# matthewdm0816/BridgeQA

Hardware: AMD Instinct MI355X
Metric: train samples/s (40k-pt scene + 512^2 view, bs16) (higher is better)
Workload: dtype bf16

## Files before the change

bridgeqa_amd/_ext.py:

```python
import ctypes
import os

import torch

_LIB_PATH = os.environ.get("BQHIP_LIB") or os.path.join(os.path.dirname(os.path.abspath(__file__)), "lib", "libbqhip.so")

if not os.path.exists(_LIB_PATH):
    raise ImportError(
        "bridgeqa_amd: %s is missing -- build it with `python -m bridgeqa_amd.build` "
        "(hipcc --offload-arch=gfx950). There is no CPU fallback." % _LIB_PATH)

_lib = ctypes.CDLL(_LIB_PATH)
_lib.bq_last_error.restype = ctypes.c_char_p
_lib.bq_abi_version.restype = ctypes.c_int
ABI_VERSION = 6
if _lib.bq_abi_version() != ABI_VERSION:
    raise ImportError("bridgeqa_amd: libbqhip.so ABI %d != %d (stale library: python -m bridgeqa_amd.build --force)"
                      % (_lib.bq_abi_version(), ABI_VERSION))

_vp, _i, _f = ctypes.c_void_p, ctypes.c_int, ctypes.c_float
_SIGS = {
    "bq_opt_n_threads": [_i],
    "bq_furthest_point_sampling": [_vp, _vp, ctypes.c_size_t, _vp, _i, _i, _i, _vp],
    "bq_furthest_point_sampling_bruteforce": [_vp, _vp, _vp, _i, _i, _i, _vp],
# ... 906 lines not shown
        n_cs = Nj if (pxc and qxc and f32) else Ni
        if epilogue != EPI_BIAS_CE and colsum is not None and (colsum.dtype != torch.float32 or colsum.numel() != n_cs
                                                               or not colsum.is_contiguous()):
            raise RuntimeError("gemm: colsum must be a contiguous fp32 (%d,) tensor" % n_cs)
        for t, nm in ((out2, "out2"), (aux, "aux")):
            if epilogue != EPI_BIAS_CE and t is not None and (t.dtype != torch.bfloat16 or t.shape != out.shape
                                                              or t.stride() != out.stride()):
                raise RuntimeError("gemm: %s must be bf16 and laid out like out" % nm)
        d.bias, d.out2, d.aux, d.colsum = _p(bias), _p(out2), _p(aux), _p(colsum)
        d.ldp, d.ldq, d.ldo = P.stride(0), ldq, ldo
        d.q_rpb, d.q_bstride, d.o_rpb, d.o_bstride = q_rpb, q_bs, o_rpb, o_bs
        d.accum = int(bool(pr.get("accum", False)))
        d.Ni, d.Nj, d.Kc = Ni, Nj, Kc
        d.p_bytes, d.q_bytes, d.ksplit = int(pr.get("p_bytes", 0)), int(pr.get("q_bytes", 0)), int(pr.get("ksplit", 1))
        if "Kc" in pr:
            d.Kc = int(pr["Kc"])
        mid_ok = (not qxc and not f32 and d.Kc >= 128 and colsum is None
                  and epilogue in (EPI_NONE, EPI_BIAS, EPI_BIAS_GELU, EPI_DGELU, EPI_ADD))
        all_mid_ok = mid_ok if k == 0 else (all_mid_ok and mid_ok)
        t_auto = max(t_auto, pick_tile(Ni, Nj, qxc, True))
    if t_auto == 128 and not all_mid_ok:
        t_auto = 256
    if (t_auto == 128 and TILE256_MIN_K[0] and not pxc and epilogue in (EPI_NONE, EPI_BIAS)
            and all(int(arr[k].Kc) >= TILE256_MIN_K[0] for k in range(n))):
        t_auto = 256
    if t_auto == 256 and any_map and tile is None and not (pxc and qxc and f32):
        t_auto = 64
    dev = problems[0]["out"].device
    if (tile or t_auto) != 128:
        flags &= ~GEMM_BACKGROUND
    with torch.cuda.device(dev):
        if (tile or t_auto) == 128 and n == 1 and (STREAMK[0] or STREAMK256[0]):
            _streamk_workspace(dev)
        _check(_lib.bq_gemm_bf16(arr, n, int(flags), int(epilogue), int(tile or t_auto), _stream()), "gemm_bf16")


def _gemm_grouped_det(problems, flags, epilogue, tile):
    if STREAMK[0] or STREAMK256[0]:
        raise RuntimeError("gemm: stream-K is on (streamk_enable / streamk256_enable) while the deterministic mode is on")
    f32 = bool(flags & GEMM_OUT_F32)
    probs, folds, sums = [], [], []
    for pr in problems:
        ks = int(pr.get("ksplit", 1))
        if epilogue != EPI_BIAS_CE and ks > 1:
            out = pr["out"]
            if not f32 or pr.get("colsum") is not None or pr.get("accum") or out.dim() != 2 or out.stride(1) != 1:
                raise RuntimeError("gemm: a cut contraction in the deterministic mode needs fp32 plain-row out, no colsum or accum")
            slab = torch.empty(ks, out.shape[0], out.stride(0), dtype=torch.float32, device=out.device)
            folds.append((slab, out, ks))
            pr = dict(pr, out=slab[0, :, :out.shape[1]])
        elif not f32 and epilogue != EPI_BIAS_CE and pr.get("colsum") is not None:
            sums.append((pr["out"], pr["colsum"]))
            pr = dict(pr, colsum=None)
        probs.append(pr)
    _gemm_grouped_launch(probs, flags | GEMM_DET, epilogue, tile)
    for slab, out, ks in folds:
        R, C = out.shape
        with torch.cuda.device(out.device):
            _check(_det_entry("gemm_splitk_fold")(_p(slab), _p(out), None, ks, R, C, out.stride(0), _stream()),
                   "gemm_splitk_fold_det")
    if sums:
        _colsum_grouped_into([o.reshape(-1, o.shape[-1]) if o.dim() == 3 else o for o, _ in sums], [c for _, c in sums],
                             "gemm_epilogue_colsum")


STREAMK = [False]
STREAMK256 = [os.environ.get("BQ_GEMM_STREAMK256", "0") == "1"]
_SK_WS = {}
_lib.bq_gemm_workspace_bytes.restype = ctypes.c_long
_lib.bq_gemm_set_workspace.argtypes = [_vp, ctypes.c_long, _vp]
_lib.bq_gemm_set_workspace.restype = ctypes.c_int
_lib.bq_gemm_streamk_mode.argtypes = [_i]
_lib.bq_gemm_streamk_mode.restype = ctypes.c_int


def _streamk_apply():
    on = STREAMK[0] or STREAMK256[0]
    _lib.bq_gemm_streamk_mode((1 if STREAMK[0] else 0) | (2 if STREAMK256[0] else 0))
    for (d, sp), (ws, st) in _SK_WS.items():
        with torch.cuda.device(d):
            _check(_lib.bq_gemm_set_workspace(_p(ws) if on else None, ws.numel() if on else 0, sp), "gemm_set_workspace")


def streamk_enable(flag):
    STREAMK[0] = bool(flag)
    _streamk_apply()


def streamk256_enable(flag):
    STREAMK256[0] = bool(flag)
    _streamk_apply()


_streamk_apply()


def _streamk_workspace(dev):
    st = torch.cuda.current_stream(dev)
    key = (dev.index if dev.index is not None else torch.cuda.current_device(), st.cuda_stream)
    if key in _SK_WS or torch.cuda.is_current_stream_capturing():
        return
    nbytes = int(_lib.bq_gemm_workspace_bytes())
    ws = torch.zeros(nbytes, dtype=torch.uint8, device=dev)
    _check(_lib.bq_gemm_set_workspace(_p(ws), nbytes, st.cuda_stream), "gemm_set_workspace")
    _SK_WS[key] = (ws, st)


def gemm_fwd(x, w, bias=None, gelu=False, tile=None, out=None, background=False):
    _mat(x, "x"), _mat(w, "w")
    M, N = x.shape[0], w.shape[0]
    with torch.cuda.device(x.device):
        y = torch.empty(M, N, dtype=torch.bfloat16, device=x.device) if out is None else out
        act = torch.empty_like(y) if gelu else None
    epi = EPI_BIAS_GELU if gelu else (EPI_BIAS if bias is not None else EPI_NONE)
    gemm_grouped([dict(P=w, Q=x, out=y, bias=bias, out2=act)], GEMM_BACKGROUND if background else 0, epi, tile)
    return (y, act) if gelu else y


def gemm_dx(dy, w, pre_act=None, colsum=None, tile=None, add=None, background=False, wt=None):
    _mat(dy, "dy"), _mat(w, "w")
    M, K = dy.shape[0], w.shape[1]
    if pre_act is not None and add is not None:
        raise RuntimeError("gemm_dx: pre_act and add are exclusive")
    if wt is not None and (colsum is not None or tuple(wt.shape) != (K, w.shape[0])):
        wt = None
    with torch.cuda.device(dy.device):
        dx = torch.empty(M, K, dtype=torch.bfloat16, device=dy.device)
    gemm_grouped([dict(P=w if wt is None else wt, Q=dy, out=dx, aux=pre_act if add is None else add, colsum=colsum)],
                 (GEMM_P_XC if wt is None else 0) | (GEMM_BACKGROUND if background else 0),
                 EPI_DGELU if pre_act is not None else (EPI_ADD if add is not None else EPI_NONE), tile)
    return dx


def gemm_dw(dy, x, tile=None):
    _mat(dy, "dy"), _mat(x, "x")
    N, K = dy.shape[1], x.shape[1]
    with torch.cuda.device(dy.device):
        dw = torch.empty(N, K, dtype=torch.float32, device=dy.device)
    gemm_grouped([dict(P=x, Q=dy, out=dw)], GEMM_P_XC | GEMM_Q_XC | GEMM_OUT_F32, EPI_NONE, tile)
    return dw


class _ColsumDesc(ctypes.Structure):
    _fields_ = [("g", _vp), ("out", _vp), ("M", _i), ("N", _i), ("ld", _i)]


_lib.bq_colsum_grouped_bf16.argtypes = [ctypes.POINTER(_ColsumDesc), _i, _vp]
_lib.bq_colsum_grouped_bf16.restype = ctypes.c_int


_lib.bq_colsum_grouped_det_floats.argtypes = [ctypes.POINTER(_ColsumDesc), _i]
_lib.bq_colsum_grouped_det_floats.restype = _l
_lib.bq_colsum_grouped_det_bf16.argtypes = [ctypes.POINTER(_ColsumDesc), _i, _vp, _vp]
_lib.bq_colsum_grouped_det_bf16.restype = ctypes.c_int


def _colsum_grouped_into(mats, outs, site):
    n = len(mats)
    arr = (_ColsumDesc * n)()
    for k, (m, o) in enumerate(zip(mats, outs)):
        _mat(m, "g")
        if m.dtype != torch.bfloat16 or o.dtype != torch.float32 or not o.is_contiguous() or o.numel() != m.shape[1]:
            raise RuntimeError("colsum_grouped: bf16 (M, N) matrices into contiguous fp32 (N,) sums")
        arr[k].g, arr[k].out, arr[k].M, arr[k].N, arr[k].ld = m.data_ptr(), o.data_ptr(), m.shape[0], m.shape[1], m.stride(0)
    dev = mats[0].device
    with torch.cuda.device(dev):
# ... 483 lines not shown
```

bridgeqa_amd/csrc/gemm_common.h:

```cpp
#pragma once
#include <type_traits>

#include "bq_common.h"
#include "bqhip_fusion.h"

namespace bq {

typedef __bf16 bf16x8 __attribute__((ext_vector_type(8)));
typedef __bf16 bf16x4 __attribute__((ext_vector_type(4)));
typedef float f32x4 __attribute__((ext_vector_type(4)));
typedef __attribute__((address_space(3))) bf16x4 lds_bf16x4_t;
typedef __attribute__((address_space(3))) void lds_void_t;

enum { EPI_NONE = 0, EPI_BIAS = 1, EPI_BIAS_GELU = 2, EPI_DGELU = 3, EPI_BIAS_CE = 4, EPI_ADD = 5 };
enum { GF_P_XC = 1, GF_Q_XC = 2, GF_OUT_F32 = 4, GF_ACCUM = 8 };

struct GemmProblem {
  const __bf16 *P, *Q;
  void *out;
  const void *bias;
  void *out2;
  const __bf16 *aux;
  float *colsum;
  int ldp, ldq, ldo;
  int Ni, Nj, Kc;
  int tile0;
  unsigned p_bytes, q_bytes;
  int q_bstride, o_bstride;
  int rpb_pack;
  int tiles_ks;
  int flags;
  __host__ __device__ __forceinline__ int q_rpb() const { return rpb_pack & 0xffff; }
  __host__ __device__ __forceinline__ int o_rpb() const { return (int)((unsigned)rpb_pack >> 16); }
  __host__ __device__ __forceinline__ int tiles_i() const { return tiles_ks & 0xffff; }
  __host__ __device__ __forceinline__ int ksplit() const { return (int)((unsigned)tiles_ks >> 16); }
  __host__ __device__ __forceinline__ int bias_bf16() const { return flags & 1; }
  __host__ __device__ __forceinline__ int accum() const { return (flags >> 1) & 1; }
};
static_assert(sizeof(GemmProblem) == 112, "GemmProblem grew: GEMM_MAX_PROBLEMS x sizeof must stay below the 4 KB kernarg limit");

__device__ __forceinline__ unsigned mapped_row(int r, int ld, int rpb, int bstride) {
  if (rpb == 0) return (unsigned)(r * ld);
  const int b = r / rpb;
  return (unsigned)(b * bstride + (r - b * rpb) * ld);
}

__device__ __forceinline__ void load_bias4(const GemmProblem &pr, int i, float (&bv)[4]) {
  if (pr.bias_bf16()) {
    const bf16x4 b = *reinterpret_cast<const bf16x4 *>(reinterpret_cast<const __bf16 *>(pr.bias) + i);
    bv[0] = (float)b[0]; bv[1] = (float)b[1]; bv[2] = (float)b[2]; bv[3] = (float)b[3];
  } else {
    const float4 b = *reinterpret_cast<const float4 *>(reinterpret_cast<const float *>(pr.bias) + i);
    bv[0] = b.x; bv[1] = b.y; bv[2] = b.z; bv[3] = b.w;
  }
}

constexpr int GEMM_MAX_PROBLEMS = 36;
struct GemmArgs {
  int n;
  int total_tiles;
  GemmProblem p[GEMM_MAX_PROBLEMS];
  void *sk_ws;
};
constexpr long SK_TICKET_BYTES = 65536, SK_SLAB_BYTES = 256 * 128 * 4;
static_assert(sizeof(GemmArgs) <= 4096, "kernel-argument limit");

__device__ __forceinline__ int xg(int kc) { return ((kc >> 1) & 1) | (((kc >> 3) & 1) << 1); }

constexpr float GELU_A1 = 1.59525515f, GELU_A3 = 7.38511083e-2f, GELU_A5 = -6.82350683e-4f;
__device__ __forceinline__ float gauss_cdf(float x, float &x2) {
  const float xc = __builtin_amdgcn_fmed3f(x, -8.0f, 8.0f);
  x2 = xc * xc;
  constexpr float L = -1.4426950408889634f;
  const float z = xc * __builtin_fmaf(x2, __builtin_fmaf(x2, GELU_A5 * L, GELU_A3 * L), GELU_A1 * L);
  return __builtin_amdgcn_rcpf(1.0f + __builtin_amdgcn_exp2f(z));
}
__device__ __forceinline__ float gelu_f(float x) {
  float x2;
  return x * gauss_cdf(x, x2);
}
__device__ __forceinline__ float dgelu_f(float x) {
  const float xc = __builtin_amdgcn_fmed3f(x, -8.0f, 8.0f);
  const float x2 = xc * xc;
  constexpr float L = -1.4426950408889634f;
  const float z = xc * __builtin_fmaf(x2, __builtin_fmaf(x2, GELU_A5 * L, GELU_A3 * L), GELU_A1 * L);
  const float s = __builtin_amdgcn_rcpf(1.0f + __builtin_amdgcn_exp2f(z));
  const float u = xc * __builtin_fmaf(x2, __builtin_fmaf(x2, 5.0f * GELU_A5, 3.0f * GELU_A3), GELU_A1);
  const float v = __builtin_fmaf(-s, s, s);
  return __builtin_fmaf(u, v, s);
}

constexpr unsigned GELU_TAB_LO = (127 - 16) << 7, GELU_TAB_HI = (127 + 3) << 7;
constexpr int GELU_TAB_HALF = (int)(GELU_TAB_HI - GELU_TAB_LO) + 1, GELU_TAB_N = 2 * GELU_TAB_HALF;
template <bool DERIV>
__device__ __forceinline__ void gelu_tab_fill(float *tab, int tid, int nthreads) {
  for (int e = tid; e < GELU_TAB_N; e += nthreads) {
    const unsigned sgn = e >= GELU_TAB_HALF ? 1u : 0u;
    const unsigned bits = (sgn << 15) | ((unsigned)e - sgn * GELU_TAB_HALF + GELU_TAB_LO);
    const float x = __uint_as_float(bits << 16);
    float x2;
    tab[e] = DERIV ? dgelu_f(x) : gauss_cdf(x, x2);
  }
}
__device__ __forceinline__ float gelu_tab_at(const float *tab, unsigned bits16) {
  const unsigned mag = min(max(bits16 & 0x7fffu, GELU_TAB_LO), GELU_TAB_HI) - GELU_TAB_LO;
  return tab[mag + ((bits16 >> 15) & 1u) * GELU_TAB_HALF];
}

template <int CTRL>
__device__ __forceinline__ float dpp_f32_add(float v) {
  return __int_as_float(__builtin_amdgcn_update_dpp(0, __float_as_int(v), CTRL, 0xF, 0xF, true));
}

__device__ __forceinline__ unsigned pack_bf16x2(float a, float b) {
  typedef __bf16 bf16x2_t __attribute__((ext_vector_type(2)));
  bf16x2_t v = {(__bf16)a, (__bf16)b};
  return __builtin_bit_cast(unsigned, v);
}

template <bool XC>
__device__ __forceinline__ bf16x8 read_frag(const unsigned char *unit, int sub16, int kk, int kc_base, const int (&xc_base)[4]) {
  if (!XC) {
    return *reinterpret_cast<const bf16x8 *>(unit + sub16 * 2048 + (kc_base ^ (kk << 6)));
  } else {
    const unsigned char *a0 = unit + xc_base[sub16] + kk * 4096;
    const bf16x4 lo = __builtin_amdgcn_ds_read_tr16_b64_v4bf16((lds_bf16x4_t *)a0);
    const bf16x4 hi = __builtin_amdgcn_ds_read_tr16_b64_v4bf16((lds_bf16x4_t *)(a0 + 512));
    return __builtin_shufflevector(lo, hi, 0, 1, 2, 3, 4, 5, 6, 7);
  }
}

template <bool XC>
__device__ __forceinline__ bf16x8 read_frag_cf(const unsigned char *unit, int sub16, int kk, int kc_base, int xc0, int xcg) {
  if (!XC) {
    return *reinterpret_cast<const bf16x8 *>(unit + sub16 * 2048 + (kc_base ^ (kk << 6)));
  } else {
    const unsigned char *a0 = unit + xc0 + ((sub16 ^ xcg) << 5) + kk * 4096;
    const bf16x4 lo = __builtin_amdgcn_ds_read_tr16_b64_v4bf16((lds_bf16x4_t *)a0);
    const bf16x4 hi = __builtin_amdgcn_ds_read_tr16_b64_v4bf16((lds_bf16x4_t *)(a0 + 512));
    return __builtin_shufflevector(lo, hi, 0, 1, 2, 3, 4, 5, 6, 7);
  }
}

template <bool XC>
__device__ __forceinline__ bf16x8 read_frag(const unsigned char *unit, int sub16, int kk, int kc_base, const int (&xc_base)[4]);
// ... 77 lines not shown
```

bridgeqa_amd/csrc/gemm_mid.hip:

```cpp
#include "gemm_common.h"

#ifndef BQ_MID_ABLATE
#define BQ_MID_ABLATE 0
#endif

namespace bq {

typedef __attribute__((address_space(3))) unsigned char lds_u8_t;
typedef unsigned u32x2_t __attribute__((ext_vector_type(2)));
typedef unsigned u32x4_t __attribute__((ext_vector_type(4)));

template <bool P_XC, bool Q_XC, int EPI, bool OUT_F32, int ST_AUX, bool SK = false>
__global__ __launch_bounds__(256, 2) void gemm128_kernel(const GemmArgs args) {
  static_assert(!OUT_F32 || (P_XC && Q_XC && EPI == EPI_NONE), "fp32 out = the weight-gradient form");
  static_assert(!Q_XC || OUT_F32, "a contraction-major Q = the weight-gradient form");
  static_assert(!SK || (!OUT_F32 && EPI != EPI_BIAS_GELU), "stream-K: bf16 out, one output");
  __shared__ __attribute__((aligned(16))) unsigned char smem[65536 + 4 * 2048 + (SK ? 16 : 0)];
  const int tid = threadIdx.x;
  const int lane = tid & 63;
  const int wave = __builtin_amdgcn_readfirstlane(tid >> 6);
  const int wr = wave >> 1, wc = wave & 1;
  const int nwg = args.total_tiles, G = (int)gridDim.x;

  const int row16 = lane & 15, q4 = lane >> 4, cp = lane & 7, lr = lane >> 3;
  const int kc_base = row16 * 128 + ((q4 ^ (row16 & 7)) << 4);
  const int xc_q = (lane & 15) >> 2;
  const int xcg = (xc_q >> 1) | ((q4 & 1) << 1), xc0 = (8 * q4 + xc_q) * 128 + 8 * (lane & 3);
  constexpr int PA0 = 0, PA1 = 16384, QB = 32768;
  const int uA0 = PA0 + wr * 8192, uA1 = PA1 + wr * 8192;
  const int bsub = wc * 2;

  struct Tile { int pi, i0, j0, nkt, kt0, t; };
  auto xcd_order = [](int v, int n) {
    const int q = n >> 3, r = n & 7, x = v & 7;
    return (x < r ? x * (q + 1) : r * (q + 1) + (x - r) * q) + (v >> 3);
  };
  auto decode_t = [&](int t) {
    int pi = 0;
    for (int k = 1; k < args.n; ++k)
      if (t >= args.p[k].tile0) pi = k;
    const GemmProblem &pr = args.p[pi];
    const int tl = t - pr.tile0;
    const int tiles_j = (pr.Nj + 127) >> 7;
    Tile tt;
    tt.pi = pi;
    tt.j0 = (tiles_j - 1 - tl / pr.tiles_i()) * 128;
    tt.i0 = (tl % pr.tiles_i()) * 256;
    tt.nkt = (pr.Kc + 63) >> 6;
    tt.kt0 = 0;
    tt.t = t;
    return tt;
  };
  auto decode = [&](int v) { return decode_t(xcd_order(v, nwg)); };
  const int nkt_full = SK ? (args.p[0].Kc + 63) >> 6 : 1;
  const int U = SK ? nwg * nkt_full : 0;
  auto bound = [&](int x) {
    int b = (int)((long)x * U / G);
    const int r = b % nkt_full;
    return r == 1 ? b - 1 : (r == nkt_full - 1 ? b + 1 : b);
  };
  auto seg = [&](int u, int ue) {
    const int t = u / nkt_full;
    Tile tt = decode_t(t);
    tt.kt0 = u - t * nkt_full;
    const int left = nkt_full - tt.kt0;
    tt.nkt = left < ue - u ? left : ue - u;
    return tt;
  };
  const int slot = SK ? xcd_order((int)blockIdx.x, G) : 0;
  int su = SK ? bound(slot) : 0;
  const int sue = SK ? bound(slot + 1) : 0;

  unsigned vP[2], vQ[2];
  unsigned stepP[2], dgP[2], ddP[2], ddQ[2], stepQ[2];
  int remP[2], remQ[2];
  int rsrcP_pi[2], rsrcQ_pi[2];
  const unsigned DEAD = 0x80000000u;
  const int ur0 = wave * 8 + lr;

  auto set_p = [&](int half, const Tile &tt, bool live) {
    const GemmProblem &pr = args.p[tt.pi];
    const int ldp = pr.ldp;
    unsigned v;
    if (!P_XC) v = (unsigned)(((tt.i0 + half * 64 + ur0) * ldp + (cp ^ (ur0 & 7)) * 8) * 2);
    else v = (unsigned)((ur0 * ldp + tt.i0 + half * 64 + (cp ^ (xg(ur0) << 1)) * 8) * 2);
    stepP[half] = P_XC ? (unsigned)(64 * ldp * 2) : 128u;
    if (SK) v += (unsigned)tt.kt0 * stepP[half];
    vP[half] = live ? v : DEAD;
    dgP[half] = P_XC ? 256u : (unsigned)(128 * ldp * 2);
    ddP[half] = (unsigned)(32 * ldp * 2);
    remP[half] = live ? tt.nkt : 0x40000000;
    rsrcP_pi[half] = tt.pi;
  };
  auto set_q = [&](int half, const Tile &tt, bool live) {
    const GemmProblem &pr = args.p[tt.pi];
    unsigned v;
    if (!Q_XC) {
      const int row0 = tt.j0 + half * 32 + ur0;
      const unsigned o0 = mapped_row(row0, pr.ldq, pr.q_rpb(), pr.q_bstride);
      v = (o0 + (unsigned)((cp ^ (ur0 & 7)) * 8)) * 2u;
      ddQ[half] = pr.q_rpb() ? (mapped_row(row0 + 64, pr.ldq, pr.q_rpb(), pr.q_bstride) - o0) * 2u : (unsigned)(64 * pr.ldq * 2);
    } else {
      const int c = cp ^ (xg(ur0) << 1);
      v = (unsigned)((ur0 * pr.ldq + tt.j0 + (c >> 2) * 64 + half * 32 + (c & 3) * 8) * 2);
      ddQ[half] = (unsigned)(32 * pr.ldq * 2);
    }
    stepQ[half] = Q_XC ? (unsigned)(64 * pr.ldq * 2) : 128u;
    if (SK) v += (unsigned)tt.kt0 * stepQ[half];
    vQ[half] = live ? v : DEAD;
    remQ[half] = live ? tt.nkt : 0x40000000;
    rsrcQ_pi[half] = tt.pi;
  };

  int v = blockIdx.x;
  Tile cur = SK ? seg(su, sue) : decode(v);
  bool has_next = SK ? (su + cur.nkt < sue) : (v + G < nwg);
  Tile nxt = has_next ? (SK ? seg(su + cur.nkt, sue) : decode(v + G)) : cur;

  auto dma_p = [&](int half) {
    const GemmProblem &pr = args.p[rsrcP_pi[half]];
    const auto rs = __builtin_amdgcn_make_buffer_rsrc((void *)pr.P, 0, pr.p_bytes, 0x00020000);
#pragma unroll
    for (int g = 0; g < 2; ++g)
#pragma unroll
      for (int d = 0; d < 2; ++d)
        if (BQ_MID_ABLATE != 2)
          __builtin_amdgcn_raw_ptr_buffer_load_lds(rs, (lds_void_t *)(smem + (half ? PA1 : PA0) + g * 8192 + (wave + 4 * d) * 1024),
                                                   16, vP[half] + (g * dgP[half] + d * ddP[half]), 0, 0, 0);
    vP[half] += stepP[half];
    if (--remP[half] == 0) set_p(half, nxt, has_next);
  };
  auto dma_q = [&](int half, unsigned par) {
    const GemmProblem &pr = args.p[rsrcQ_pi[half]];
    const auto rs = __builtin_amdgcn_make_buffer_rsrc((void *)pr.Q, 0, pr.q_bytes, 0x00020000);
#pragma unroll
    for (int d = 0; d < 2; ++d)
// ... 274 lines not shown
#pragma unroll
      for (int b = 0; b < 4; ++b) {
#pragma unroll
        for (int pass = 0; pass < NPASS; ++pass) {
#pragma unroll
          for (int half = 0; half < 2; ++half) {
#pragma unroll
            for (int a4 = 0; a4 < 4; ++a4) {
              const int a = half * 4 + a4;
              float vv[4];
#pragma unroll
              for (int r = 0; r < 4; ++r) vv[r] = (float)(__bf16)acc[a][b][r];
              if (EPI == EPI_BIAS_GELU && pass == 1) {
#pragma unroll
                for (int r = 0; r < 4; ++r) vv[r] = gelu_f(vv[r]);
              }
              const u32x2_t pk = {pack_bf16x2(vv[0], vv[1]), pack_bf16x2(vv[2], vv[3])};
              asm volatile("ds_write_b64 %0, %1" ::"v"(ep_lds + (unsigned)(wj + (((a4 * 2 + wc2) ^ wx) << 4))), "v"(pk) : "memory");
            }
            asm volatile("s_waitcnt lgkmcnt(0)" ::: "memory");
            __builtin_amdgcn_sched_barrier(0);
            u32x4_t d[2];
#pragma unroll
            for (int t2 = 0; t2 < 2; ++t2) {
              const int jr = t2 * 8 + lr;
              asm volatile("ds_read_b128 %0, %1" : "=v"(d[t2]) : "v"(ep_lds + (unsigned)(jr * 128 + ((cp ^ (jr & 7)) << 4))) : "memory");
            }
            asm volatile("s_waitcnt lgkmcnt(0)" : "+v"(d[0]), "+v"(d[1])::"memory");
            __builtin_amdgcn_sched_barrier(0);
#pragma unroll
            for (int t2 = 0; t2 < 2; ++t2) {
              const int i_st = iw + half * 64 + cp * 8;
              const unsigned off = i_st < Ni ? (jrow[b][t2] + (unsigned)i_st) * 2u : DEAD;
              __builtin_amdgcn_raw_buffer_store_b128(d[t2], pass == 1 ? rsO2 : rsO, off, 0, ST_AUX);
            }
          }
        }
      }
    }

    if (SK) {
      su += cur.nkt;
      if (su >= sue) break;
      cur = nxt;
      has_next = su + cur.nkt < sue;
      if (has_next) nxt = seg(su + cur.nkt, sue);
    } else {
      v += G;
      if (v >= nwg) break;
      cur = nxt;
      has_next = v + G < nwg;
      if (has_next) nxt = decode(v + G);
    }
  }
  asm volatile("s_waitcnt vmcnt(0)" ::: "memory");
}

struct SkWorkspace { int device; hipStream_t stream; void *ptr; long bytes; };
static SkWorkspace g_sk_ws[16];
static int g_sk_n = 0;

void *gemm_sk_workspace(hipStream_t st, long *bytes) {
  int dev = 0;
  if (hipGetDevice(&dev) != hipSuccess) return nullptr;
  for (int i = 0; i < g_sk_n; ++i)
    if (g_sk_ws[i].device == dev && g_sk_ws[i].stream == st) {
      *bytes = g_sk_ws[i].bytes;
      return g_sk_ws[i].ptr;
    }
  return nullptr;
}

static int g_sk_mode = 0;
int gemm_sk_mode() {
  static int env_off = -1;
  if (env_off < 0) {
    const char *e = getenv("BQ_GEMM_STREAMK");
    env_off = (e != nullptr && e[0] == '0') ? 1 : 0;
  }
  return env_off ? 0 : g_sk_mode;
}
static bool sk_enabled() { return (gemm_sk_mode() & 1) != 0; }

int launch_gemm_mid(const GemmArgs &ga_in, bool p_xc, bool q_xc, bool out_f32, int epi, bool background, hipStream_t stream) {
  const int slots = 2 * device_cus();
  for (int k = 0; k < ga_in.n; ++k)
    if (ga_in.p[k].Kc < 128) return -1;
  GemmArgs ga = ga_in;
  ga.sk_ws = nullptr;
  if (sk_enabled() && !background && ga.n == 1 && !p_xc && !q_xc && !out_f32 && (epi == EPI_NONE || epi == EPI_BIAS || epi == EPI_ADD)) {
    const int nkt = (ga.p[0].Kc + 63) >> 6, tiles = ga.total_tiles;
    const long units = (long)tiles * nkt;
    const int rounds = (tiles + slots - 1) / slots;
    long ws_bytes = 0;
    void *ws = gemm_sk_workspace(stream, &ws_bytes);
    if (ws != nullptr && nkt >= 24 && tiles >= slots / 2 && units / slots >= 16 && (long)rounds * nkt * slots >= units * 115 / 100
        && 8L * tiles <= SK_TICKET_BYTES && ws_bytes >= SK_TICKET_BYTES + 2L * slots * SK_SLAB_BYTES) {
      ga.sk_ws = ws;
      const dim3 grid(slots), block(256);
      if (epi == EPI_NONE) hipLaunchKernelGGL((gemm128_kernel<false, false, EPI_NONE, false, 16, true>), grid, block, 0, stream, ga);
      else if (epi == EPI_BIAS) hipLaunchKernelGGL((gemm128_kernel<false, false, EPI_BIAS, false, 16, true>), grid, block, 0, stream, ga);
      else hipLaunchKernelGGL((gemm128_kernel<false, false, EPI_ADD, false, 16, true>), grid, block, 0, stream, ga);
      return 0;
    }
  }
  const int use = background ? (slots + 1) / 2 : slots;
  const dim3 grid(ga.total_tiles < use ? ga.total_tiles : use), block(256);
#define BQ_MID_LAUNCH(PX, E)                                                                                        \
  do {                                                                                                              \
    hipLaunchKernelGGL((gemm128_kernel<PX, false, E, false, 16>), grid, block, 0, st_, ga);                         \
    return 0;                                                                                                       \
  } while (0)
  hipStream_t st_ = stream;
  if (q_xc || out_f32) {
    if (!(p_xc && q_xc && out_f32 && epi == EPI_NONE)) return -1;
    hipLaunchKernelGGL((gemm128_kernel<true, true, EPI_NONE, true, 16>), grid, block, 0, st_, ga);
    return 0;
  }
  for (int k = 0; k < ga.n; ++k)
    if (ga.p[k].colsum != nullptr) return -1;
  if (!p_xc) {
    if (epi == EPI_NONE) BQ_MID_LAUNCH(false, EPI_NONE);
    if (epi == EPI_BIAS) BQ_MID_LAUNCH(false, EPI_BIAS);
    if (epi == EPI_BIAS_GELU) BQ_MID_LAUNCH(false, EPI_BIAS_GELU);
    if (epi == EPI_DGELU) BQ_MID_LAUNCH(false, EPI_DGELU);
    if (epi == EPI_ADD) BQ_MID_LAUNCH(false, EPI_ADD);
  } else {
    if (epi == EPI_NONE) BQ_MID_LAUNCH(true, EPI_NONE);
    if (epi == EPI_DGELU) BQ_MID_LAUNCH(true, EPI_DGELU);
    if (epi == EPI_ADD) BQ_MID_LAUNCH(true, EPI_ADD);
  }
  return -1;
}

}

extern "C" int bq_gemm_streamk_mode(int mode) {
  const int old = bq::g_sk_mode;
  if (mode >= 0) bq::g_sk_mode = mode & 3;
  return old;
}

extern "C" long bq_gemm_workspace_bytes(void) {
  return bq::SK_TICKET_BYTES + 2L * 2L * bq::device_cus() * bq::SK_SLAB_BYTES;
}

extern "C" int bq_gemm_set_workspace(void *ws, long bytes, void *stream) {
  using namespace bq;
  int dev = 0;
  BQ_REQUIRE(hipGetDevice(&dev) == hipSuccess, BQ_EINVAL, "bq_gemm_set_workspace: no device");
  BQ_REQUIRE(ws == nullptr || bytes >= bq_gemm_workspace_bytes(), BQ_EINVAL, "bq_gemm_set_workspace: %ld bytes < %ld", bytes,
             bq_gemm_workspace_bytes());
  for (int i = 0; i < g_sk_n; ++i)
    if (g_sk_ws[i].device == dev && g_sk_ws[i].stream == (hipStream_t)stream) {
      g_sk_ws[i].ptr = ws;
      g_sk_ws[i].bytes = bytes;
      return 0;
    }
  BQ_REQUIRE(g_sk_n < 16, BQ_ELIMIT, "bq_gemm_set_workspace: more than 16 (device, stream) pairs");
  g_sk_ws[g_sk_n++] = SkWorkspace{dev, (hipStream_t)stream, ws, bytes};
  return 0;
}
```

include/bqhip_fusion.h:

```cpp
#ifndef BQHIP_FUSION_H
#define BQHIP_FUSION_H
#include "bqhip.h"

#ifdef __cplusplus
extern "C" {
#endif

BQ_API int bq_attn_fwd(const void *Q, const void *K, const void *V, void *O, float *LSE, const float *mask, int B,
                       int H, int Lq, int Lk, int Lkp, long q_bs, long q_rs, long q_hs, long k_bs, long k_rs,
                       long k_hs, long o_bs, long o_rs, long o_hs, float scale, float p_drop, unsigned seed,
                       const unsigned *seed_ptr, int causal, void *stream);

BQ_API int bq_attn_bwd(const void *Q, const void *K, const void *V, const void *dO, const float *LSE, const void *O,
                       float *DELTA, const float *mask, void *dQ, void *dK, void *dV, int B, int H, int Lq, int Lk,
                       int Lkp, long q_bs, long q_rs, long q_hs, long k_bs, long k_rs, long k_hs, long g_bs, long g_rs,
                       long g_hs, float scale, float p_drop, unsigned seed, const unsigned *seed_ptr, int causal,
                       void *stream);

typedef struct bq_attn_side {
  const void *Q, *K, *V, *dO, *O;
  void *out, *dK, *dV;
  float *LSE, *DELTA;
  const float *mask;
  int Lq, Lk, Lkp;
// ... 73 lines not shown
                                 const float *rstd, float *partial, float *dgb, long R, int C, int S, int relu, int pool,
                                 void *stream);
BQ_API int bq_bn_backward_reduce_arg(const void *dy, const void *x, const void *arg, const float *scale, const float *shift,
                                     const float *mean, const float *rstd, float *partial, float *dgb, long R, int C, int S,
                                     int relu, void *stream);
BQ_API int bq_sa_bwd_supported(int ldx, int Nj, int S, int pool, int need_dx);
BQ_API int bq_sa_bwd_workgroups(long R, int ldx, int Nj, int pool, int need_dx);
BQ_API int bq_sa_bwd_fused(const void *x, const void *p, const void *dout, const void *arg, const void *w, const float *scale,
                           const float *shift, const float *mean, const float *rstd, const float *dgb, void *dx, float *dw,
                           float *part, long R, int ldx, int Nj, int ldw, int ldo, int S, int relu, int pool, void *stream);
BQ_API int bq_pwconv_bn_fwd_x(const void *x, const float *xscale, const float *xshift, long R, int K, int ldx, const void *w,
                              int ldw, int Kc, int N, void *y, float *partial, const float *gamma, const float *beta,
                              float *running_mean, float *running_var, long long *num_batches_tracked, float eps,
                              float momentum, float *scale, float *shift, float *mean, float *rstd, const float *center,
                              float *shift_acc, void *stream);
BQ_API int bq_sa_bwd_reduce_supported(int ldx, int Nj, int S, int pool);
BQ_API int bq_sa_bwd_fused_xr(const void *x, const float *xscale, const float *xshift, const float *xmean, const float *xrstd,
                              float *red_part, float *red_dgb, const void *p, const void *dout, const void *arg, const void *w,
                              const float *scale, const float *shift, const float *mean, const float *rstd, const float *dgb,
                              void *dx, float *dw, float *part, long R, int ldx, int Nj, int ldw, int ldo, int S, int relu,
                              int pool, void *stream);
BQ_API int bq_sa_bwd_fused_x(const void *x, const float *xscale, const float *xshift, const void *p, const void *dout,
                             const void *arg, const void *w, const float *scale, const float *shift, const float *mean,
                             const float *rstd, const float *dgb, void *dx, float *dw, float *part, long R, int ldx, int Nj,
                             int ldw, int ldo, int S, int relu, int pool, void *stream);

BQ_API int bq_gelu_fwd_bf16(const void *x, void *y, long n, void *stream);
BQ_API int bq_twin_drop_add_ln_fwd(const void *x, const void *residual, const float *gamma, const float *beta,
                                   const float *gamma2, const float *beta2, void *y, float *mean, float *rstd,
                                   float *zero_out, int M, int H, float eps, float p_drop, unsigned seed,
                                   const unsigned *seed_ptr, void *stream);
BQ_API int bq_twin_drop_add_ln_bwd(const void *x, const void *residual, const float *gamma, const float *gamma2,
                                   const void *dy, const float *mean, const float *rstd, void *dx, void *dresidual,
                                   float *dgb, int M, int H, float eps, float p_drop, unsigned seed,
                                   const unsigned *seed_ptr, void *stream);

BQ_API int bq_adamw_chunk_elems(void);
BQ_API int bq_adamw_tensor_bytes(void);
BQ_API int bq_adamw_multi(const void *table, const void *chunks, int n_chunks, const float *step, float beta1,
                          float beta2, float eps, float grad_clip_value, void *stream);

BQ_API int bq_box_point_count(const float *points, const float *center, const float *size, const float *heading, int *count,
                              int B, int N, int ld, int K, int cap, void *stream);
BQ_API int bq_nms(const float *box, const float *score, const int *cls, const unsigned char *valid, unsigned char *keep,
                  int B, int K, float thresh, int old_type, int same_cls, void *stream);

BQ_API int bq_project_points(const float *points, const float *depth, const float *frames, int *pix, int F, int N, int W,
                             int H, float fx, float fy, float cx, float cy, float depth_min, float depth_max,
                             float accuracy, void *stream);
BQ_API int bq_fuse_point_features(const int *pix, const float *feat, float *out, int F, int N, int HW, int C, int maxpool,
                                  void *stream);

#define BQ_GEMM_P_XC 1
#define BQ_GEMM_Q_XC 2
#define BQ_GEMM_OUT_F32 4
#define BQ_GEMM_BACKGROUND 8
#define BQ_GEMM_DET 16
#define BQ_GEMM_EPI_NONE 0
#define BQ_GEMM_EPI_BIAS 1
#define BQ_GEMM_EPI_BIAS_GELU 2
#define BQ_GEMM_EPI_DGELU 3
#define BQ_GEMM_EPI_ADD 5
#define BQ_GEMM_EPI_BIAS_CE 4
typedef struct bq_gemm_desc {
  const void *P, *Q;
  void *out;
  const float *bias;
  void *out2;
  const void *aux;
  float *colsum;
  int ldp, ldq, ldo;
  int Ni, Nj, Kc;
  int bias_bf16;
  long p_bytes, q_bytes;
  int ksplit;
  int q_rpb, q_bstride, o_rpb, o_bstride;
  int accum;
} bq_gemm_desc;
BQ_API int bq_gemm_max_problems(void);
BQ_API int bq_gemm_bf16(const bq_gemm_desc *problems, int n, int flags, int epilogue, int tile, void *stream);
BQ_API long bq_gemm_workspace_bytes(void);
BQ_API int bq_gemm_set_workspace(void *ws, long bytes, void *stream);
BQ_API int bq_gemm_streamk_mode(int mode);

typedef struct bq_colsum_desc {
  const void *g;
  float *out;
  int M, N, ld;
} bq_colsum_desc;
BQ_API int bq_colsum_grouped_bf16(const bq_colsum_desc *problems, int n, void *stream);
BQ_API long bq_colsum_grouped_det_floats(const bq_colsum_desc *problems, int n);
BQ_API int bq_colsum_grouped_det_bf16(const bq_colsum_desc *problems, int n, float *partial, void *stream);
BQ_API int bq_gemm_splitk_fold_det(const float *slab, float *out, void *out_bf16, int pieces, int rows, int cols, int ld,
                                   void *stream);

BQ_API int bq_transpose_tensor_bytes(void);
BQ_API int bq_transpose_multi_bf16(const void *table, const void *chunks, int n_chunks, int max_wgs, void *stream);

BQ_API int bq_wgrad_rows_supported(int Ni, int Nj);
BQ_API int bq_wgrad_rows_workgroups(long R, int Ni, int Nj, int workgroups);
BQ_API int bq_wgrad_rows_bf16(const void *P, const void *Q, float *out, float *part, long R, int Ni, int Nj, int ldp,
                              int ldq, int ldo, int workgroups, void *stream);

BQ_API int bq_pwconv_records(long R, int N);
BQ_API int bq_pwconv_bn_fwd(const void *x, long R, int K, int ldx, const void *w, int ldw, int Kc, int N, void *y,
                            float *partial, const float *gamma, const float *beta, float *running_mean,
                            float *running_var, long long *num_batches_tracked, float eps, float momentum,
                            float *scale, float *shift, float *mean, float *rstd, const float *center, float *shift_acc,
                            void *stream);
BQ_API int bq_pwconv_bn_apply(const void *x, long R, int K, int ldx, const void *w, int ldw, int Kc, int N, const float *scale,
                              const float *shift_acc, void *out, int S, int relu, int pool, void *stream);

BQ_API int bq_lmhead_ce_combine(const float *partial, const float *target_logit, const int *target, float *loss,
                                float *lse, int R, int nrec, int V, float label_smoothing, void *stream);
BQ_API int bq_lmhead_ce_dlogits(void *logits, const float *lse, const int *target, const float *grad_loss, int R, int V,
                                int ld, float label_smoothing, void *stream);

BQ_API size_t bq_invert_index_workspace_bytes(long total);
BQ_API int bq_invert_index(const int32_t *idx, int B, long L, int N, int32_t *start, unsigned *slots, void *workspace,
                           size_t workspace_bytes, void *stream);
BQ_API int bq_group_concat_pm_grad_gather(const void *grad_out, int in_bf16, const int32_t *start, const unsigned *slots,
                                          float *grad_feats, float *grad_xyz, float *grad_new_xyz, int B, int C, int N, int M,
                                          int S, int ld, float radius, int normalize, void *stream);
BQ_API int bq_three_interpolate_grad_gather(const float *grad_out, const int32_t *start, const unsigned *slots,
                                            const float *weight, float *grad_points, int B, int C, int n, int m, void *stream);

typedef struct bq_det_loss_desc {
  const float *seed_xyz, *vote_xyz, *aggregated_vote_xyz, *objectness_scores, *center, *heading_scores,
      *heading_residuals_normalized, *size_scores, *size_residuals_normalized, *sem_cls_scores;
  const void *seed_inds;
  const float *vote_label;
  const void *vote_label_mask;
  const float *center_label, *box_label_mask;
  const void *heading_class_label, *size_class_label, *sem_cls_label;
  const float *heading_residual_label, *size_residual_label, *mean_size_arr;
  float *terms;
  void *objectness_label;
  float *objectness_mask;
  void *object_assignment;
  float *g_vote_xyz, *g_objectness_scores, *g_center, *g_heading_scores, *g_heading_residuals_normalized, *g_size_scores,
      *g_size_residuals_normalized, *g_sem_cls_scores;
  int *scratch;
  int B, S, VF, N, K, G, NH, NS, NC;
  int cl_ld;
  int seed_inds_i64;
  int ld_objectness_scores, ld_heading_scores, ld_heading_residuals_normalized, ld_size_scores, ld_size_residuals_normalized,
      ld_sem_cls_scores;
  float near_threshold, far_threshold, objectness_weight_neg, objectness_weight_pos;
} bq_det_loss_desc;
BQ_API int bq_det_loss_fwd(const bq_det_loss_desc *d, void *stream);
typedef struct bq_det_loss_seg {
  const float *g;
  float *out;
  int rows, width, ld, term;
} bq_det_loss_seg;
BQ_API int bq_det_loss_bwd(const bq_det_loss_seg *segments, int n, const float *upstream, void *stream);

typedef struct bq_mlp_eval_layer {
  const void *w;
  const float *gamma, *beta, *mean, *var, *bias;
  float eps;
  int n, ldw, relu;
} bq_mlp_eval_layer;
typedef struct bq_mlp_eval_desc {
  const float *xyz, *new_xyz, *feats;
  long f_bs, f_rs;
// ... 22 lines not shown
```

Measured before the change: 501.3.

## Group GEMM tiles along i for L2 reuse with XCD-aware run assignment

Adds a tile-ordering plan for the mid GEMM kernel. For single-problem launches where P is the weight, tiles are grouped into bands along i so each band's P panel fits a byte budget, and the ordering reuses it across j tiles. XCD run start offsets are chosen so group boundaries line up with dispatch rounds. The plan uses a cost model and a 256-mask search on the host. It adds a TileOrder to the kernel args and extra decode arithmetic per tile on the device.

```diff
diff --git a/bridgeqa_amd/_ext.py b/bridgeqa_amd/_ext.py
--- a/bridgeqa_amd/_ext.py
+++ b/bridgeqa_amd/_ext.py
@@ -1012,6 +1012,12 @@
             _check(_lib.bq_gemm_set_workspace(_p(ws) if on else None, ws.numel() if on else 0, sp), "gemm_set_workspace")
 
 
+def gemm_tile_order(mode=-1, budget_bytes=-1):
+    _lib.bq_gemm_tile_order.argtypes = [_i, ctypes.c_long]
+    _lib.bq_gemm_tile_order.restype = ctypes.c_int
+    return _lib.bq_gemm_tile_order(int(mode), int(budget_bytes))
+
+
 def streamk_enable(flag):
     STREAMK[0] = bool(flag)
     _streamk_apply()
diff --git a/bridgeqa_amd/csrc/gemm_common.h b/bridgeqa_amd/csrc/gemm_common.h
--- a/bridgeqa_amd/csrc/gemm_common.h
+++ b/bridgeqa_amd/csrc/gemm_common.h
@@ -3,6 +3,7 @@
 
 #include "bq_common.h"
 #include "bqhip_fusion.h"
+#include "gemm_tile_order.h"
 
 namespace bq {
 
@@ -61,6 +62,7 @@
   int total_tiles;
   GemmProblem p[GEMM_MAX_PROBLEMS];
   void *sk_ws;
+  TileOrder ord;
 };
 constexpr long SK_TICKET_BYTES = 65536, SK_SLAB_BYTES = 256 * 128 * 4;
 static_assert(sizeof(GemmArgs) <= 4096, "kernel-argument limit");
diff --git a/bridgeqa_amd/csrc/gemm_mid.hip b/bridgeqa_amd/csrc/gemm_mid.hip
--- a/bridgeqa_amd/csrc/gemm_mid.hip
+++ b/bridgeqa_amd/csrc/gemm_mid.hip
@@ -31,27 +31,24 @@
   const int bsub = wc * 2;
 
   struct Tile { int pi, i0, j0, nkt, kt0, t; };
-  auto xcd_order = [](int v, int n) {
-    const int q = n >> 3, r = n & 7, x = v & 7;
-    return (x < r ? x * (q + 1) : r * (q + 1) + (x - r) * q) + (v >> 3);
-  };
+  auto xcd_order = [](int v, int n) { return tile_order_xcd(v, n); };
+  const int ord_groups = SK ? 1 : args.ord.groups, ord_flags = SK ? 0 : args.ord.flags;
   auto decode_t = [&](int t) {
     int pi = 0;
     for (int k = 1; k < args.n; ++k)
       if (t >= args.p[k].tile0) pi = k;
     const GemmProblem &pr = args.p[pi];
-    const int tl = t - pr.tile0;
-    const int tiles_j = (pr.Nj + 127) >> 7;
+    const TilePos tp = tile_order_decode(t - pr.tile0, pr.tiles_i(), (pr.Nj + 127) >> 7, ord_groups, ord_flags);
     Tile tt;
     tt.pi = pi;
-    tt.j0 = (tiles_j - 1 - tl / pr.tiles_i()) * 128;
-    tt.i0 = (tl % pr.tiles_i()) * 256;
+    tt.j0 = tp.bj * 128;
+    tt.i0 = tp.bi * 256;
     tt.nkt = (pr.Kc + 63) >> 6;
     tt.kt0 = 0;
     tt.t = t;
     return tt;
   };
-  auto decode = [&](int v) { return decode_t(xcd_order(v, nwg)); };
+  auto decode = [&](int v) { return decode_t(tile_order_position(args.ord, v)); };
   const int nkt_full = SK ? (args.p[0].Kc + 63) >> 6 : 1;
   const int U = SK ? nwg * nkt_full : 0;
   auto bound = [&](int x) {
@@ -492,6 +489,9 @@
 }
 static bool sk_enabled() { return (gemm_sk_mode() & 1) != 0; }
 
+static int g_tile_order_mode = 0;
+static long g_tile_order_budget = TILE_ORDER_BUDGET_BYTES;
+
 int launch_gemm_mid(const GemmArgs &ga_in, bool p_xc, bool q_xc, bool out_f32, int epi, bool background, hipStream_t stream) {
   const int slots = 2 * device_cus();
   for (int k = 0; k < ga_in.n; ++k)
@@ -516,6 +516,8 @@
   }
   const int use = background ? (slots + 1) / 2 : slots;
   const dim3 grid(ga.total_tiles < use ? ga.total_tiles : use), block(256);
+  tile_order_for_launch(ga.ord, ga.n, ga.total_tiles, (int)grid.x, ga.p[0].tiles_i(), (ga.p[0].Nj + 127) >> 7, ga.p[0].Kc,
+                        !out_f32 && !q_xc, g_tile_order_mode, g_tile_order_budget);
 #define BQ_MID_LAUNCH(PX, E)                                                                                        \
   do {                                                                                                              \
     hipLaunchKernelGGL((gemm128_kernel<PX, false, E, false, 16>), grid, block, 0, st_, ga);                         \
@@ -551,6 +553,14 @@
   return old;
 }
 
+extern "C" int bq_gemm_tile_order(int mode, long budget_bytes) {
+  const int old = bq::g_tile_order_mode;
+  if (mode >= 0 && mode <= 2) bq::g_tile_order_mode = mode;
+  if (budget_bytes > 0) bq::g_tile_order_budget = budget_bytes;
+  if (budget_bytes == 0) bq::g_tile_order_budget = bq::TILE_ORDER_BUDGET_BYTES;
+  return old;
+}
+
 extern "C" long bq_gemm_workspace_bytes(void) {
   return bq::SK_TICKET_BYTES + 2L * 2L * bq::device_cus() * bq::SK_SLAB_BYTES;
 }
diff --git a/bridgeqa_amd/csrc/gemm_tile_order.h b/bridgeqa_amd/csrc/gemm_tile_order.h
--- /dev/null
+++ b/bridgeqa_amd/csrc/gemm_tile_order.h
@@ -0,0 +1,120 @@
+#pragma once
+
+#if defined(__HIPCC__)
+#define BQ_TO_HD __host__ __device__ inline
+#else
+#define BQ_TO_HD inline
+#endif
+
+namespace bq {
+
+constexpr int TILE_ORDER_LABELS = 8;
+constexpr long TILE_ORDER_BUDGET_BYTES = 6L * 256 * 768 * 2;
+enum { TILE_ORDER_J_FASTEST = 1 };
+
+struct TileOrder {
+  int start[TILE_ORDER_LABELS];
+  int groups;
+  int flags;
+};
+
+struct TilePos { int bi, bj; };
+
+BQ_TO_HD int tile_order_run_start(int x, int total) {
+  const int q = total >> 3, r = total & 7;
+  return x < r ? x * (q + 1) : r * (q + 1) + (x - r) * q;
+}
+BQ_TO_HD int tile_order_xcd(int v, int total) { return tile_order_run_start(v & 7, total) + (v >> 3); }
+
+BQ_TO_HD int tile_order_group_width(int g, int tiles_i, int groups) { return tiles_i / groups + (g < tiles_i % groups ? 1 : 0); }
+
+BQ_TO_HD int tile_order_groups(int tiles_i, int tiles_j, int rows_i, int rows_j, int Kc, int total, int grid, long budget) {
+  if (tiles_i < 2 || grid < 1 || Kc < 1) return 1;
+  long per = budget / (2L * rows_i * Kc);
+  if (per < 1) per = 1;
+  if (tiles_i <= per) return 1;
+  const int groups = (int)((tiles_i + per - 1) / per);
+  const long rounds = (total + grid - 1) / grid;
+  const long Ri = (long)tiles_i * rows_i, Rj = (long)tiles_j * rows_j;
+  return groups * Rj + TILE_ORDER_LABELS * Ri < Rj + TILE_ORDER_LABELS * rounds * Ri ? groups : 1;
+}
+
+BQ_TO_HD TilePos tile_order_decode(int tl, int tiles_i, int tiles_j, int groups, int flags) {
+  int bi, jr;
+  if (flags & TILE_ORDER_J_FASTEST) {
+    bi = tl / tiles_j;
+    jr = tl - bi * tiles_j;
+  } else if (groups <= 1) {
+    jr = tl / tiles_i;
+    bi = tl - jr * tiles_i;
+  } else {
+    const int base = tiles_i / groups, wide = tiles_i % groups;
+    const int big = wide * (base + 1) * tiles_j;
+    int w, i0, r;
+    if (tl < big) {
+      w = base + 1;
+      const int g = tl / (w * tiles_j);
+      r = tl - g * w * tiles_j;
+      i0 = g * w;
+    } else {
+      w = base;
+      const int g = (tl - big) / (w * tiles_j);
+      r = tl - big - g * w * tiles_j;
+      i0 = wide * (base + 1) + g * w;
+    }
+    jr = r / w;
+    bi = i0 + (r - jr * w);
+  }
+  TilePos p;
+  p.bi = bi;
+  p.bj = tiles_j - 1 - jr;
+  return p;
+}
+
+BQ_TO_HD void tile_order_plan(TileOrder &o, int total, int grid, int groups, int tiles_i, int tiles_j, int flags) {
+  o.groups = 1;
+  o.flags = flags;
+  for (int x = 0; x < TILE_ORDER_LABELS; ++x) o.start[x] = tile_order_run_start(x, total);
+  if (groups <= 1 || (flags & TILE_ORDER_J_FASTEST) || grid < 8 || (grid & 7) != 0 || grid >= total || tiles_i * tiles_j != total ||
+      groups > tiles_i)
+    return;
+  o.groups = groups;
+  const int q = total >> 3, r = total & 7, set = grid >> 3;
+  int best_mask = 0, best_cost = 1 << 30;
+  for (int mask = 0; mask < 256; ++mask) {
+    int bits = 0;
+    for (int s = 0; s < 8; ++s) bits += (mask >> s) & 1;
+    if (bits != r) continue;
+    int cost = 0, edge = 0;
+    for (int g = 0; g + 1 < groups; ++g) {
+      edge += tile_order_group_width(g, tiles_i, groups) * tiles_j;
+      int s0 = 0;
+      for (int s = 0; s < 8; ++s) {
+        const int len = q + ((mask >> s) & 1);
+        if (edge > s0 && edge < s0 + len) cost += (edge - s0) % set != 0 ? 16 : 1;
+        s0 += len;
+      }
+    }
+    if (cost < best_cost) {
+      best_cost = cost;
+      best_mask = mask;
+    }
+  }
+  int s0 = 0, nl = 0, ns = r;
+  for (int s = 0; s < 8; ++s) {
+    const int lng = (best_mask >> s) & 1;
+    o.start[lng ? nl++ : ns++] = s0;
+    s0 += q + lng;
+  }
+}
+
+BQ_TO_HD void tile_order_for_launch(TileOrder &o, int nproblems, int total, int grid, int tiles_i, int tiles_j, int Kc,
+                                    bool p_is_weight, int mode, long budget) {
+  int groups = 1;
+  if (mode == 0 && nproblems == 1 && p_is_weight) groups = tile_order_groups(tiles_i, tiles_j, 256, 128, Kc, total, grid, budget);
+  tile_order_plan(o, total, grid, groups, tiles_i, tiles_j, mode == 2 && nproblems == 1 ? (int)TILE_ORDER_J_FASTEST : 0);
+}
+
+BQ_TO_HD int tile_order_position(const TileOrder &o, int v) { return o.start[v & 7] + (v >> 3); }
+
+}
diff --git a/include/bqhip_fusion.h b/include/bqhip_fusion.h
--- a/include/bqhip_fusion.h
+++ b/include/bqhip_fusion.h
@@ -179,6 +179,7 @@
 BQ_API long bq_gemm_workspace_bytes(void);
 BQ_API int bq_gemm_set_workspace(void *ws, long bytes, void *stream);
 BQ_API int bq_gemm_streamk_mode(int mode);
+BQ_API int bq_gemm_tile_order(int mode, long budget_bytes);
 
 typedef struct bq_colsum_desc {
   const void *g;
```

Measured after the change: 500.8. Within noise of the previous version (-0.1%).
